# Traneptora/hydrium

Measured on AMD Instinct MI355X. Metric: Mpixel/s encode (8K RGB, default q), higher is better.
Workload: dtype f32

## Files before the change

### hydrium_amd/csrc/hip/device_api.hip

```cpp
#include <hip/hip_runtime.h>

#include <stdint.h>
#include <stdio.h>
#include <stdlib.h>
#include <string.h>

#include <atomic>
#include <condition_variable>
#include <functional>
#include <mutex>
#include <thread>
#include <vector>

#include "../../../include/hydrium_amd.h"
#include "hydk_common.h"
#include "../hyd_sample_fmt.h"

#pragma clang fp contract(off)

namespace hydk {
hipError_t launch_transform(const HydkLfJob *d_jobs, int num_slots, unsigned fmt_mask, int xmode, uint32_t *status,
                            uint2 *part_info, int plog, hipStream_t stream);
hipError_t launch_tables(const uint32_t *hist, HydkTables *tabs, const uint32_t *alpha_max, int nclusters, int first_slot,
                         int num_slots, uint32_t alpha_floor, const uint32_t *alpha_floor_dev, const uint32_t *lf_hist,
// ... 5 lines not shown
hipError_t launch_rans(const HydkLfJob *d_jobs, const uint32_t *sym_count, const HydkTables *tabs, uint32_t *bitbuf,
                       uint32_t bit_pitch_words, uint32_t *group_bits, int num_slots, const uint32_t *status,
                       hipStream_t stream);
hipError_t launch_rans_deferred(const HydkLfJob *d_jobs, const uint32_t *sym_count, const HydkTables *tabs, uint16_t *aux,
                                uint16_t *flags, uint32_t aux_pitch, uint32_t *final_state, uint32_t *group_bits,
                                int num_slots, const uint32_t *status, hipStream_t stream);
hipError_t launch_rans_lanes(const HydkLfJob *d_jobs, const uint32_t *sym_count, const HydkTables *tabs, uint16_t *aux,
                             uint16_t *flags, uint32_t aux_pitch, uint32_t *final_state, uint32_t *group_bits,
                             int nclusters, int num_slots, const uint32_t *status, const uint32_t *lf_hist,
                             HydkLfStream *lf_streams, void *lf_work, hipStream_t stream);
hipError_t launch_lf_front(const HydkLfJob *d_jobs, unsigned long long *recs, uint32_t *hist, void *work, int num_slots,
                           hipStream_t stream);
hipError_t launch_lf_back(const HydkLfJob *d_jobs, const unsigned long long *recs, HydkLfStream *streams, uint32_t *bits,
                          void *work, int num_slots, hipStream_t stream);
hipError_t launch_rans_emit(const HydkLfJob *d_jobs, const uint32_t *sym_count, const uint16_t *aux, const uint16_t *flags,
                            uint32_t aux_pitch, const uint32_t *final_state, const uint32_t *group_bits, const uint64_t *offsets,
                            uint8_t *payload, int num_slots, const uint32_t *status, hipStream_t stream);
hipError_t launch_frame_begin(const HydkLfJob *host_jobs, HydkLfJob *d_jobs, int count, uint32_t *accum, size_t accum_words,
                              hipStream_t stream);
hipError_t launch_publish(const uint64_t *total, uint64_t *h_total, const unsigned long long *lf_total,
                          unsigned long long *h_lf_total, const uint32_t *status, uint32_t *h_status, hipStream_t stream);
hipError_t transform_footprint(int fmt, int storage, int xmode, int *lds_bytes, int *registers);
hipError_t launch_scan(const uint32_t *group_bits, int count, uint64_t *offsets, uint64_t *total, uint8_t *payload,
                       uint64_t payload_cap, int clear_shared_words, uint32_t *status, hipStream_t stream);
hipError_t launch_pack(const uint32_t *bitbuf, uint32_t bit_pitch_words, const uint32_t *group_bits, const uint64_t *offsets,
                       uint8_t *payload, int count, const uint32_t *status, hipStream_t stream);
size_t lf_work_bytes();
hipError_t launch_batch_extents(const void *blob, int frames, void *extents, hipStream_t stream);
hipError_t launch_lf_coder(const HydkLfJob *d_jobs, unsigned long long *recs, uint32_t *hist, HydkLfStream *streams,
                           uint32_t *bits, void *work, int num_slots, hipStream_t stream);
hipError_t launch_lf_gather(HydkLfStream *streams, const uint32_t *bits, uint32_t *packed, unsigned long long *total,
                            int num_slots, hipStream_t stream);
// ... 43 lines not shown
    int linear_light = 0;
    int use_luts = 2;
    int best_register_mode = 2;
    int curve_gathers = 0;
    uint64_t published_pixels = 0;
    uint64_t seen_bytes = 0, seen_pixels = 0;
    int register_luts_ok = 0;
    int rans_lanes = 0;
    uint32_t tok_cap = HYDK_DEFAULT_TOKEN_CAP;
    bool caps_forced = false;
    unsigned grown_ahead = 0;
    uint32_t rec_bytes = 4;
    uint32_t bit_pitch_words = 0;
    int want_transform = 0, want_entropy = 0;
    bool slot_lanes[HYDAMD_MAX_LF_GROUPS] = {};
    unsigned overflow_reruns = 0;
    uint32_t alpha_floor = 0;
    const uint32_t *alpha_floor_dev = nullptr;
    unsigned num_presets = 1;
    int scheme = 0;
    int nclusters = 9;
    hipStream_t own_stream = nullptr;
    hipStream_t stream = nullptr;
    char error[256] = "";

    char *tokens = nullptr;
    uint32_t *bitbuf = nullptr;
    uint16_t *rans_aux = nullptr;
    uint16_t *rans_flags = nullptr;
    uint32_t *rans_final = nullptr;
// ... 1975 lines not shown
                                                 ctx->lf_streams + first, ctx->lf_work + (size_t)first * hydk::lf_work_bytes(),
                                                 ctx->stream));
        } else if (!any_float && wave_form_defers()) {
            HIP_TRY(ctx, hydk::launch_rans_deferred(jobs, ctx->sym_count + g0, ctx->tables + first, ctx->rans_aux + g0 * ctx->tok_cap,
                                                    ctx->rans_flags + g0 * (ctx->tok_cap / 16), ctx->tok_cap, ctx->rans_final + g0,
                                                    ctx->group_bits + g0, count, ctx->status, ctx->stream));
            emits = true;
        } else {
            const int st = ensure_bitbuf(ctx);
            if (st != ST_OK)
                return st;
            HIP_TRY(ctx, hydk::launch_rans(jobs, ctx->sym_count + g0, ctx->tables + first,
                                           ctx->bitbuf + g0 * ctx->bit_pitch_words, ctx->bit_pitch_words,
                                           ctx->group_bits + g0, count, ctx->status, ctx->stream));
        }
        for (int i = first; i < first + count; i++)
            ctx->slot_lanes[i] = emits;
    }
    return ST_OK;
}

int hydamd_run_entropy(HydAmdContext *ctx, int num_slots) {
    if (!ctx)
        return ST_API_ERROR;
    if (num_slots < 1 || num_slots > ctx->max_slots)
        return fail(ctx, ST_API_ERROR, "slot count out of range");
    if (num_slots > ctx->transformed)
        return fail(ctx, ST_API_ERROR, "the entropy stage needs the transform stage of the same slots first");
    HIP_TRY(ctx, hipSetDevice(ctx->device));
    const int count = num_slots * HYDK_GROUPS_PER_LFG;
    ctx->results_valid = false;
    ctx->want_entropy = num_slots;
// ... 9 lines not shown
            ScopedTimer timer(ctx, HYDAMD_K_LF);
            if (!(lf_drop() & 1))
            HIP_TRY(ctx, hydk::launch_lf_front(ctx->d_jobs + lf_first, ctx->lf_recs + (size_t)lf_first * HYDK_LF_SYMBOLS,
                                               ctx->lf_hist + (size_t)lf_first * HYDK_LF_CODES,
                                               ctx->lf_work + (size_t)lf_first * hydk::lf_work_bytes(), lf_count, ctx->stream));
        }
    }
    if (num_slots > ctx->coded) {
        const int st = entropy_range(ctx, ctx->coded, num_slots - ctx->coded, lf_count > 0 && !(lf_drop() & 2));
        if (st != ST_OK)
            return st;
        ctx->coded = num_slots;
    }
    if (!(debug_skip() & 4)) {
        ScopedTimer timer(ctx, HYDAMD_K_PACK);
        HIP_TRY(ctx, hydk::launch_scan(ctx->group_bits, count, ctx->offsets, ctx->total, ctx->payload, ctx->payload_cap, 1,
                                       ctx->status, ctx->stream));
        for (int first = 0; first < num_slots;) {
            int last = first;
            while (last + 1 < num_slots && ctx->slot_lanes[last + 1] == ctx->slot_lanes[first])
                last++;
            const int n = last - first + 1;
            const size_t g0 = (size_t)first * HYDK_GROUPS_PER_LFG;
            if (ctx->slot_lanes[first])
                HIP_TRY(ctx, hydk::launch_rans_emit(ctx->d_jobs + first, ctx->sym_count + g0, ctx->rans_aux + g0 * ctx->tok_cap,
                                                    ctx->rans_flags + g0 * (ctx->tok_cap / 16), ctx->tok_cap,
                                                    ctx->rans_final + g0, ctx->group_bits + g0, ctx->offsets + g0, ctx->payload,
                                                    n, ctx->status, ctx->stream));
            else
                HIP_TRY(ctx, hydk::launch_pack(ctx->bitbuf + g0 * ctx->bit_pitch_words, ctx->bit_pitch_words,
                                               ctx->group_bits + g0, ctx->offsets + g0, ctx->payload,
                                               n * HYDK_GROUPS_PER_LFG, ctx->status, ctx->stream));
            first = last + 1;
        }
    }
    if (lf_count > 0) {
        ScopedTimer timer(ctx, HYDAMD_K_LF);
        if (!(lf_drop() & 4))
        HIP_TRY(ctx, hydk::launch_lf_back(ctx->d_jobs + lf_first, ctx->lf_recs + (size_t)lf_first * HYDK_LF_SYMBOLS,
                                          ctx->lf_streams + lf_first, ctx->lf_bits + (size_t)lf_first * HYDK_LF_BITWORDS,
                                          ctx->lf_work + (size_t)lf_first * hydk::lf_work_bytes(), lf_count, ctx->stream));
        ctx->lf_coded = num_slots;
        ctx->lf_need_gather = true;
// ... 322 lines not shown
    if (run_pairs)
        *run_pairs = h.run_pairs;
    if (bit_count)
        *bit_count = h.bit_count;
    return ST_OK;
}

int hydamd_read_lf_bits(HydAmdContext *ctx, int slot, uint8_t *dst, size_t capacity) {
    int st = check_slot(ctx, slot);
    if (st != ST_OK)
        return st;
    if (!ctx->lf_on_device || !ctx->lf_results_valid)
        return fail(ctx, ST_API_ERROR, "no device-coded LF stream: the LF coder is off or the frame was not synchronised");
    if (capacity > (size_t)HYDK_LF_BITWORDS * sizeof(uint32_t))
        return fail(ctx, ST_API_ERROR, "LF bit request too large");
    if (capacity)
        HIP_TRY(ctx, hipMemcpy(dst, ctx->lf_bits + (size_t)slot * HYDK_LF_BITWORDS, capacity, hipMemcpyDeviceToHost));
    return ST_OK;
}

size_t hydamd_lf_payload_size(HydAmdContext *ctx) {
    return ctx && ctx->lf_results_valid && ctx->lf_on_device ? (size_t)ctx->h_lf_total : 0;
}

const uint8_t *hydamd_lf_payload_device(HydAmdContext *ctx) { return ctx ? (const uint8_t *)ctx->lf_packed : nullptr; }

int hydamd_read_lf_payload(HydAmdContext *ctx, uint8_t *dst, size_t capacity) {
    if (!ctx || !ctx->lf_on_device || !ctx->lf_results_valid)
        return fail(ctx, ST_API_ERROR, "no device-coded LF stream: the LF coder is off or the frame was not synchronised");
    if (capacity < ctx->h_lf_total)
        return fail(ctx, ST_API_ERROR, "LF payload buffer too small");
    if (ctx->h_lf_total)
// ... 159 lines not shown
```

### hydrium_amd/csrc/hip/kernels.hip

```cpp
#include <hip/hip_runtime.h>
#include <stdint.h>

#include "hydk_common.h"
#include <atomic>
#include <type_traits>

#pragma clang fp contract(off)

namespace {

constexpr int kThreads = 256;
#ifndef HYDK_K1_WAVES
#define HYDK_K1_WAVES 4
#endif
#ifndef HYDK_K1_GATHER
#define HYDK_K1_GATHER 0x10
#endif
#ifndef HYDK_K1_WAVELOCAL
#define HYDK_K1_WAVELOCAL 1
#endif
#ifndef HYDK_K1_SKIP
#define HYDK_K1_SKIP 0
#endif
#ifndef HYDK_K1_ILP
// ... 1148 lines not shown
        if (bogus)
            atomicOr(status, HYDK_STATUS_INCONSISTENT);
    }
}

__global__ __launch_bounds__(kThreads) void k_build_tables(const uint32_t *hist_all, HydkTables *tabs,
                                                           const uint32_t *alpha_max_all, int nclusters,
                                                           uint32_t alpha_floor, const uint32_t *alpha_floor_dev,
                                                           int first_slot, int num_slots, const uint32_t *lf_hist,
                                                           HydkLfStream *lf_streams, void *lf_work, const HydkLfJob *__restrict__ jobs_all) {
    HYDK_URGENT();
    if ((int)blockIdx.x >= num_slots) {
        __shared__ LfHuffScratch s_huff;
        const int s = (int)blockIdx.x - num_slots;
        if (threadIdx.x < 64)
            lf_huffman_wave(lf_hist + (size_t)s * HYDK_LF_CODES, ((LfWork *)lf_work)[s].codes, lf_streams + s, s_huff, (int)threadIdx.x);
        return;
    }
    const unsigned slot = (unsigned)first_slot + blockIdx.x;
    const uint32_t *hist = hist_all + (size_t)slot * HYDK_MAX_CLUSTERS * HYDK_ALPHABET;
    HydkTables *tab = tabs + slot;
    __shared__ uint32_t s_freq[HYDK_MAX_CLUSTERS][HYDK_ALPHABET];
    __shared__ uint32_t s_cutoff[HYDK_MAX_CLUSTERS][HYDK_ALPHABET];
    __shared__ uint32_t s_other[HYDK_MAX_CLUSTERS][HYDK_ALPHABET];
    __shared__ uint32_t s_shift[HYDK_MAX_CLUSTERS][HYDK_ALPHABET];
    __shared__ uint32_t s_base[HYDK_MAX_CLUSTERS][HYDK_ALPHABET];
    __shared__ uint8_t s_under[HYDK_MAX_CLUSTERS][HYDK_ALPHABET];
    __shared__ uint8_t s_over[HYDK_MAX_CLUSTERS][HYDK_ALPHABET];
    __shared__ uint32_t s_alpha[HYDK_MAX_CLUSTERS];
    __shared__ uint32_t s_log_alpha, s_err;

// ... 527 lines not shown
    unsigned char *const s_tab = s_mem + kOpsBytes;
    __builtin_amdgcn_s_setprio(HYDK_CHAIN_PRIO);
#if HYDK_CHAIN_DYN_LDS
    if ((uint32_t)(uintptr_t)(__attribute__((address_space(3))) unsigned char *)s_mem != 0u)
        __builtin_trap();
#endif
#if HYDK_CHAIN_PROBE & 32
    const uint32_t probe_t0 = (uint32_t)__builtin_amdgcn_s_memrealtime();
#endif
#if HYDK_CHAIN_HOG
    asm volatile("v_accvgpr_write_b32 a255, 0" ::: "a255");
#endif
    const int lane = threadIdx.x;
    if ((int)blockIdx.x >= num_slots) {
        const int s = (int)blockIdx.x - num_slots;
        lf_huffman_wave(lf_hist + (size_t)s * HYDK_LF_CODES, ((LfWork *)lf_work)[s].codes, lf_streams + s, *(LfHuffScratch *)s_mem, lane);
        return;
    }
    const int slot = blockIdx.x;
    const int ngroups = jobs[slot].gcols * jobs[slot].grows;
    const HydkTables *tab = tabs + slot;
    if (*status & HYDK_STATUS_OVERFLOW)
        return;
    typedef __attribute__((address_space(3))) const uint16_t LdsU16;
    {
#if HYDK_LANE_TAB_GLOBAL
        const uint32_t tab_lds = 0;
#else
        const uint4 *src = (const uint4 *)&tab->inv1[0][0];
        for (int i = lane; i < NC * HYDK_ANS_SLOTS / 8; i += 64)
            ((uint4 *)s_tab)[i] = src[i];
// ... 384 lines not shown
#if HYDK_CHAIN_PROBE & 32
    if (lane == 0)
        group_bits_all[G] = probe_t0;
    if (lane == 1)
        group_bits_all[G] = (uint32_t)__builtin_amdgcn_s_memrealtime();
#endif
}

#ifndef HYDK_EMIT_SHARE_DEFAULT
#define HYDK_EMIT_SHARE_DEFAULT 1
#endif
constexpr int kEmitPer = 8;
constexpr int kEmitBatch = 64 * kEmitPer;
constexpr int kEmitWin = kEmitBatch + 4;

__global__ __launch_bounds__(kThreads) void k_rans_emit(const HydkLfJob *__restrict__ jobs, const uint32_t *sym_count_all,
                                                        const uint16_t *aux_all, const uint16_t *flags_all, uint32_t aux_pitch,
                                                        const uint32_t *final_state_all, const uint32_t *group_bits_all,
                                                        const uint64_t *offsets_all, uint8_t *payload,
                                                        const uint32_t *status, int vblocks) {
    __shared__ uint32_t s_win[4][kEmitWin];
    HYDK_URGENT();
    const int t = threadIdx.x, lane = t & 63, wave = t >> 6;
    auto one_block = [&](const int vb) {
    const int slot = vb >> 4;
    const int g = ((vb & 15) << 2) + wave;
    const int ngroups = jobs[slot].gcols * jobs[slot].grows;
    const size_t G = (size_t)slot * HYDK_GROUPS_PER_LFG + g;
    if (g >= ngroups || (*status & HYDK_STATUS_OVERFLOW))
        return;
    const void *tok = (const char *)jobs[slot].tokens + (size_t)g * jobs[slot].tok_cap * jobs[slot].rec_bytes;
    const uint4 *aux = (const uint4 *)(aux_all + G * aux_pitch);
    const uint16_t *flags = flags_all + G * (aux_pitch / 16);
    uint32_t *W = (uint32_t *)payload;
    uint32_t *win = s_win[wave];
    const int n = __builtin_amdgcn_readfirstlane((int)sym_count_all[G]);
    const uint32_t bits = group_bits_all[G];
    const unsigned long long lo_bit = offsets_all[G] * 8ull, hi_bit = lo_bit + (unsigned long long)((bits + 7u) & ~7u);
    const uint32_t shared_lo = (lo_bit & 31ull) ? (uint32_t)(lo_bit >> 5) : 0xFFFFFFFFu;
    const uint32_t shared_hi = (hi_bit & 31ull) ? (uint32_t)((hi_bit - 1ull) >> 5) : 0xFFFFFFFFu;
    const uint32_t wbase = (uint32_t)(lo_bit >> 5);
    uint32_t cur = (uint32_t)(lo_bit & 31ull) + bits;
    uint32_t carry = 0;

    bool bad = false;
    auto put = [&](uint32_t word, uint32_t v) {
        const uint32_t d = wbase + word;
        if (d == shared_lo || d == shared_hi)
            atomicOr(&W[d], v);
        else
            W[d] = v;
    };
    auto emit = [&](const uint32_t (&val)[kEmitPer], const uint32_t (&nb)[kEmitPer], auto &&before_stores) {
        uint32_t mine = 0;
#pragma unroll
        for (int j = 0; j < kEmitPer; j++)
            mine += nb[j];
        const uint32_t inc = scan64_inclusive(mine);
        const uint32_t total = __builtin_amdgcn_readlane(inc, 63);
        if (!total) {
            before_stores();
            return;
        }
        if (total > cur) {
            if (lane == 0)
                atomicOr((uint32_t *)status, HYDK_STATUS_INCONSISTENT);
            bad = true;
            return;
        }
        const uint32_t newcur = cur - total;
        const uint32_t wlo = newcur >> 5, whi = (cur - 1u) >> 5;
        const uint32_t nwords = whi - wlo + 1u;
        for (uint32_t i = lane; i < nwords; i += 64)
            win[i] = 0;
        __builtin_amdgcn_wave_barrier();
        if (lane == 0 && (cur & 31u))
            win[whi - wlo] = carry;
        __builtin_amdgcn_wave_barrier();
        uint32_t pos = newcur + (inc - mine) - wlo * 32u;
#pragma unroll
        for (int j = 0; j < kEmitPer; j++) {
// ... 416 lines not shown
    if (nclusters == 9)
        HYDK_LAUNCH_LANES(HYDK_LANE_NC9_PROBE);
    else if (nclusters == 3)
        HYDK_LAUNCH_LANES(3);
    else if (nclusters == 2)
        HYDK_LAUNCH_LANES(2);
    else if (nclusters == 1)
        HYDK_LAUNCH_LANES(1);
    else
        return hipErrorInvalidValue;
#undef HYDK_LAUNCH_LANES
    return hipGetLastError();
}

hipError_t launch_rans_emit(const HydkLfJob *d_jobs, const uint32_t *sym_count, const uint16_t *aux, const uint16_t *flags,
                            uint32_t aux_pitch, const uint32_t *final_state, const uint32_t *group_bits, const uint64_t *offsets,
                            uint8_t *payload, int num_slots, const uint32_t *status, hipStream_t stream) {
    static const int share = [] {
        const char *v = getenv("HYDAMD_EMIT_SHARE");
        const int n = v && *v ? atoi(v) : HYDK_EMIT_SHARE_DEFAULT;
        return n < 1 ? 1 : n > 16 ? 16 : n;
    }();
    const int vblocks = num_slots * 16;
    hipLaunchKernelGGL(k_rans_emit, dim3((vblocks + share - 1) / share), dim3(kThreads), 0, stream, d_jobs, sym_count, aux, flags,
                       aux_pitch, final_state, group_bits, offsets, payload, status, vblocks);
    return hipGetLastError();
}

hipError_t launch_frame_begin(const HydkLfJob *host_jobs, HydkLfJob *d_jobs, int count, uint32_t *accum, size_t accum_words,
                              hipStream_t stream) {
    const uint32_t quads = accum ? (uint32_t)(accum_words / 4) : 0u;
    const uint32_t job_words = (uint32_t)((size_t)count * sizeof(HydkLfJob) / sizeof(uint32_t));
    const uint32_t blocks = 1u + (quads + kThreads - 1) / kThreads;
    hipLaunchKernelGGL(k_frame_begin, dim3(blocks < 64u ? blocks : 64u), dim3(kThreads), 0, stream, (const uint32_t *)host_jobs,
                       (uint32_t *)d_jobs, job_words, (uint4 *)accum, quads);
    return hipGetLastError();
}

hipError_t launch_publish(const uint64_t *total, uint64_t *h_total, const unsigned long long *lf_total,
                          unsigned long long *h_lf_total, const uint32_t *status, uint32_t *h_status, hipStream_t stream) {
// ... 40 lines not shown
```

### hydrium_amd/csrc/hip/lf_coder.hip

```cpp
#include <hip/hip_runtime.h>

#include <stdint.h>

#include "hydk_common.h"
#ifndef HYDK_LF_WPB
#define HYDK_LF_WPB 1
#endif
#ifndef HYDK_LF_PROBE
#define HYDK_LF_PROBE 0
#endif

namespace {

#include "lf_huffman.h"

constexpr int kPlane = HYDK_DC_PITCH * HYDK_DC_PITCH;

#define LF_REC(v, lit, r) ((unsigned long long)(v) | ((unsigned long long)((uint32_t)(lit) | ((uint32_t)(r) << 1)) << 32))

struct LfShape {
    int vbw, blocks, n;
    uint32_t vbw_magic;
};

__device__ __forceinline__ LfShape lf_shape(const HydkLfJob &job) {
    LfShape sh;
    sh.vbw = (job.width + 7) >> 3;
    sh.blocks = sh.vbw * ((job.height + 7) >> 3);
    sh.n = 3 * sh.blocks;
    sh.vbw_magic = sh.vbw > 1 ? (uint32_t)(0xFFFFFFFFu / (uint32_t)sh.vbw) + 1u : 0u;
    return sh;
}

__device__ __forceinline__ int lf_row_of(const LfShape &sh, int rem) {
    return sh.vbw > 1 ? (int)__umulhi((uint32_t)rem, sh.vbw_magic) : rem;
}

__device__ __forceinline__ void lf_hybrid(uint32_t v, uint32_t &token, uint32_t &nbits, uint32_t &residue) {
    if (v < 128u) {
        token = v;
        nbits = 0;
        residue = 0;
        return;
    }
    const uint32_t nb = (31u - (uint32_t)__clz(v)) - 2u;
    residue = (v >> 1) & ((1u << nb) - 1u);
    token = 128u + (((nb - 5u) << 2) | (((v >> (nb + 1u)) & 1u) << 1) | (v & 1u));
    nbits = nb;
}

#define LF_DPP_KEEP(v, ctrl, rmask) ((uint32_t)__builtin_amdgcn_update_dpp((int)(v), (int)(v), ctrl, rmask, 0xF, false))
#define LF_DPP_ZERO(v, ctrl, rmask) ((uint32_t)__builtin_amdgcn_update_dpp(0, (int)(v), ctrl, rmask, 0xF, false))

__device__ __forceinline__ int wave_incl_max(int v) {
    int t;
    t = (int)LF_DPP_KEEP(v, 0x111, 0xF);
    v = v > t ? v : t;
    t = (int)LF_DPP_KEEP(v, 0x112, 0xF);
    v = v > t ? v : t;
    t = (int)LF_DPP_KEEP(v, 0x114, 0xF);
    v = v > t ? v : t;
    t = (int)LF_DPP_KEEP(v, 0x118, 0xF);
    v = v > t ? v : t;
    t = (int)LF_DPP_KEEP(v, 0x142, 0xA);
    v = v > t ? v : t;
    t = (int)LF_DPP_KEEP(v, 0x143, 0xC);
    v = v > t ? v : t;
    return v;
}

__device__ __forceinline__ uint32_t wave_incl_sum(uint32_t v) {
    v += LF_DPP_ZERO(v, 0x111, 0xF);
    v += LF_DPP_ZERO(v, 0x112, 0xF);
    v += LF_DPP_ZERO(v, 0x114, 0xF);
    v += LF_DPP_ZERO(v, 0x118, 0xF);
    v += LF_DPP_ZERO(v, 0x142, 0xA);
    v += LF_DPP_ZERO(v, 0x143, 0xC);
    return v;
}

struct LfTokenScratch {
    int wtot[kLfWaves];
    uint32_t lastv[kLfWaves];
    int head[kLfWaves];
    uint32_t first;
};

__device__ __forceinline__ uint32_t lf_predict(int32_t cur, int32_t w, int32_t n, int32_t nw) {
    const int32_t lo = w < n ? w : n, hi = w < n ? n : w;
    int32_t pred = (int32_t)((uint32_t)w + (uint32_t)n - (uint32_t)nw);
    pred = pred < lo ? lo : pred > hi ? hi : pred;
    const uint32_t d = (uint32_t)cur - (uint32_t)pred;
// ... 235 lines not shown
    const HydkLfJob &job = jobs[slot];
    const LfShape sh = lf_shape(job);
    __shared__ __attribute__((aligned(16))) int s_rs[kScanSpan];
    __shared__ uint32_t s_hist[HYDK_LF_CODES];
    __shared__ LfTokenScratch s_tok;
    __shared__ uint32_t s_rbits;
    if (HYDK_LF_PROBE & 8)
        return;
    for (int win = (int)blockIdx.x * HYDK_LF_WPB; win < ((int)blockIdx.x + 1) * HYDK_LF_WPB && win < kMaxWindows; win++) {
        const int tb = win * kEmitSpan;
        if (tb >= sh.n)
            return;
        if (tid == 0)
            s_rbits = 0;
        uint32_t rb = lf_tokens_window(job, sh, recs_all + (size_t)slot * HYDK_LF_SYMBOLS, tb, s_rs, s_hist, s_tok);
        rb = wave_incl_sum(rb);
        if ((tid & 63) == 63 && rb)
            atomicAdd(&s_rbits, rb);
        __syncthreads();
        LfWork &w = work[slot];
        for (int i = tid; i < HYDK_LF_CODES && !(HYDK_LF_PROBE & 2); i += kLfThreads) {
            const uint32_t c = s_hist[i];
            w.win_hist[win][i] = (uint16_t)c;
            if (c)
                atomicAdd(&hist_all[(size_t)slot * HYDK_LF_CODES + i], c);
        }
        if (tid == 0)
            w.win_residue_bits[win] = s_rbits;
        if (HYDK_LF_WPB > 1)
            __syncthreads();
    }
}

__global__ __launch_bounds__(64) void k_lf_codes(const uint32_t *__restrict__ hist_all, HydkLfStream *__restrict__ streams,
                                                 LfWork *__restrict__ work) {
    if (!(HYDK_LF_PROBE & 1))
        __builtin_amdgcn_s_setprio(3);
    __shared__ LfHuffScratch s_huff;
    const int slot = blockIdx.x;
    lf_huffman_wave(hist_all + (size_t)slot * HYDK_LF_CODES, work[slot].codes, streams + slot, s_huff, (int)threadIdx.x);
}

__global__ __launch_bounds__(kLfThreads) void k_lf_offsets(const HydkLfJob *__restrict__ jobs, LfWork *__restrict__ work,
                                                           HydkLfStream *__restrict__ streams, uint32_t *__restrict__ bits_all) {
    if (!(HYDK_LF_PROBE & 1))
        __builtin_amdgcn_s_setprio(3);
    const int slot = blockIdx.x, tid = threadIdx.x, lane = tid & 63, wave = tid >> 6;
    const LfShape sh = lf_shape(jobs[slot]);
    const int windows = (sh.n + kEmitSpan - 1) / kEmitSpan;
    LfWork &w = work[slot];
    __shared__ uint32_t s_win[kMaxWindows];
    __shared__ uint32_t s_wsum[kLfWaves];
    uint32_t len6[6];
#pragma unroll
    for (int j = 0; j < 6; j++)
        len6[j] = w.codes[j * 64 + lane] >> 16;
    for (int win = wave; win < windows; win += kLfWaves) {
        uint32_t bits = 0;
#pragma unroll
        for (int j = 0; j < 6; j++)
            bits += (uint32_t)w.win_hist[win][j * 64 + lane] * len6[j];
        bits = wave_incl_sum(bits);
        if (lane == 63)
            s_win[win] = bits + w.win_residue_bits[win];
    }
    __syncthreads();
    const uint32_t mine = tid < windows ? s_win[tid] : 0u;
    const uint32_t inc = wave_incl_sum(mine);
    if (lane == 63)
        s_wsum[wave] = inc;
    __syncthreads();
    uint32_t off = inc - mine, total = 0;
    for (int k = 0; k < kLfWaves; k++) {
        if (k < wave)
            off += s_wsum[k];
        total += s_wsum[k];
    }
    uint32_t *out = bits_all + (size_t)slot * HYDK_LF_BITWORDS;
    if (tid < windows) {
        w.win_off[tid] = off;
        if (mine) {
            out[off >> 5] = 0;
            out[(off + mine - 1u) >> 5] = 0;
        }
    }
    if (tid == 0)
        streams[slot].bit_count = total;
}

__global__ __launch_bounds__(kLfThreads) void k_lf_pack(const HydkLfJob *__restrict__ jobs,
                                                        const unsigned long long *__restrict__ recs_all,
                                                        const LfWork *__restrict__ work, uint32_t *__restrict__ bits_all) {
    if (!(HYDK_LF_PROBE & 1))
        __builtin_amdgcn_s_setprio(3);
    const int slot = blockIdx.y, tid = threadIdx.x, lane = tid & 63, wave = tid >> 6;
    const LfShape sh = lf_shape(jobs[slot]);
    __shared__ uint32_t s_bits[kPackWords];
    __shared__ uint32_t s_code[HYDK_LF_CODES];
    __shared__ uint32_t s_wsum[kLfWaves];
    if ((int)blockIdx.x * HYDK_LF_WPB * kEmitSpan >= sh.n)
        return;
    for (int i = tid; i < HYDK_LF_CODES; i += kLfThreads)
        s_code[i] = work[slot].codes[i];
  for (int win = (int)blockIdx.x * HYDK_LF_WPB; win < ((int)blockIdx.x + 1) * HYDK_LF_WPB && win < kMaxWindows; win++) {
    const int tb = win * kEmitSpan;
    if (tb >= sh.n)
        return;
    if (win != (int)blockIdx.x * HYDK_LF_WPB)
        __syncthreads();
    for (int w = tid; w < kPackWords; w += kLfThreads)
        s_bits[w] = 0;
    __syncthreads();
    unsigned long long val[4];
    uint32_t len[4];
    const uint32_t mine = lf_window_strings(sh, recs_all + (size_t)slot * HYDK_LF_SYMBOLS, tb, s_code, val, len);
    const uint32_t inc = wave_incl_sum(mine);
    if (lane == 63)
        s_wsum[wave] = inc;
    __syncthreads();
    const uint32_t gbits = work[slot].win_off[win];
    uint32_t pos = (gbits & 31u) + inc - mine, total = 0;
    for (int w = 0; w < kLfWaves; w++) {
        const uint32_t t = s_wsum[w];
        if (w < wave)
            pos += t;
        total += t;
    }
#pragma unroll
    for (int j = 0; j < 4; j++) {
        if (!len[j])
            continue;
        const uint32_t w = pos >> 5, shl = pos & 31u;
        const unsigned long long lo = val[j] << shl;
        const uint32_t hi = shl ? (uint32_t)(val[j] >> (64u - shl)) : 0u;
        if ((uint32_t)lo)
            atomicOr(&s_bits[w], (uint32_t)lo);
        if ((uint32_t)(lo >> 32))
            atomicOr(&s_bits[w + 1], (uint32_t)(lo >> 32));
        if (hi)
            atomicOr(&s_bits[w + 2], hi);
        pos += len[j];
    }
    __syncthreads();
    if (!total)
        continue;
    const uint32_t end = (gbits & 31u) + total, last = (end - 1u) >> 5;
    uint32_t *dst = bits_all + (size_t)slot * HYDK_LF_BITWORDS + (gbits >> 5);
    for (uint32_t w = tid; w <= last; w += kLfThreads) {
        if (w == 0 || w == last)
            atomicOr(&dst[w], s_bits[w]);
        else
            dst[w] = s_bits[w];
    }
  }
}

__global__ __launch_bounds__(256) void k_lf_gather(HydkLfStream *__restrict__ streams, const uint32_t *__restrict__ bits_all,
                                                   uint32_t *__restrict__ packed, unsigned long long *__restrict__ total,
                                                   int num_slots) {
    const int slot = blockIdx.x, tid = threadIdx.x;
    __shared__ uint32_t s_off;
    if (tid < 64) {
        uint32_t mine = 0;
        for (int s = tid; s < slot; s += 64)
            mine += (streams[s].bit_count + 31u) >> 5;
#pragma unroll
        for (int d = 32; d >= 1; d >>= 1)
// ... 4 lines not shown
    __syncthreads();
    const uint32_t off = s_off, words = (streams[slot].bit_count + 31u) >> 5;
    const uint32_t *src = bits_all + (size_t)slot * HYDK_LF_BITWORDS;
    for (uint32_t w = tid; w < words; w += 256)
        packed[off + w] = src[w];
    if (tid == 0) {
        streams[slot].offset = off * 4u;
        if (slot == num_slots - 1)
            *total = (unsigned long long)(off + words) * 4ull;
    }
}

__global__ __launch_bounds__(64) void k_lf_huffman(const uint32_t *__restrict__ hist, HydkLfStream *__restrict__ stream_out,
                                                   uint32_t *__restrict__ codes) {
    __shared__ LfHuffScratch s_huff;
    lf_huffman_wave(hist, codes, stream_out, s_huff, (int)threadIdx.x);
}

}

namespace hydk {

size_t lf_work_bytes() { return sizeof(LfWork); }

hipError_t launch_lf_front(const HydkLfJob *d_jobs, unsigned long long *recs, uint32_t *hist, void *work, int num_slots,
                           hipStream_t stream) {
    hipLaunchKernelGGL(k_lf_tokens, dim3((kMaxWindows + HYDK_LF_WPB - 1) / HYDK_LF_WPB, num_slots), dim3(kLfThreads), 0, stream, d_jobs, recs, hist, (LfWork *)work);
    return hipGetLastError();
}

hipError_t launch_lf_codes(const uint32_t *hist, HydkLfStream *streams, void *work, int num_slots, hipStream_t stream) {
    hipLaunchKernelGGL(k_lf_codes, dim3(num_slots), dim3(64), 0, stream, hist, streams, (LfWork *)work);
    return hipGetLastError();
}

hipError_t launch_lf_back(const HydkLfJob *d_jobs, const unsigned long long *recs, HydkLfStream *streams, uint32_t *bits,
                          void *work, int num_slots, hipStream_t stream) {
    LfWork *w = (LfWork *)work;
    hipLaunchKernelGGL(k_lf_offsets, dim3(num_slots), dim3(kLfThreads), 0, stream, d_jobs, w, streams, bits);
    hipLaunchKernelGGL(k_lf_pack, dim3((kMaxWindows + HYDK_LF_WPB - 1) / HYDK_LF_WPB, num_slots), dim3(kLfThreads), 0, stream, d_jobs, recs, w, bits);
    return hipGetLastError();
}

hipError_t launch_lf_coder(const HydkLfJob *d_jobs, unsigned long long *recs, uint32_t *hist, HydkLfStream *streams,
                           uint32_t *bits, void *work, int num_slots, hipStream_t stream) {
    hipError_t e = launch_lf_front(d_jobs, recs, hist, work, num_slots, stream);
    if (e == hipSuccess)
        e = launch_lf_codes(hist, streams, work, num_slots, stream);
    if (e == hipSuccess)
        e = launch_lf_back(d_jobs, recs, streams, bits, work, num_slots, stream);
    return e;
}

hipError_t launch_lf_gather(HydkLfStream *streams, const uint32_t *bits, uint32_t *packed, unsigned long long *total,
                            int num_slots, hipStream_t stream) {
    hipLaunchKernelGGL(k_lf_gather, dim3(num_slots), dim3(256), 0, stream, streams, bits, packed, total, num_slots);
    return hipGetLastError();
}

hipError_t launch_lf_huffman_only(const uint32_t *hist, HydkLfStream *stream_out, uint32_t *codes, hipStream_t stream) {
    hipLaunchKernelGGL(k_lf_huffman, dim3(1), dim3(64), 0, stream, hist, stream_out, codes);
    return hipGetLastError();
}
// ... 3 lines not shown
```

### hydrium_amd/csrc/hip/lf_huffman.h

```cpp
#ifndef HYDK_LF_HUFFMAN_H_
#define HYDK_LF_HUFFMAN_H_

constexpr int kLfThreads = 256;
constexpr int kLfWaves = kLfThreads / 64;
constexpr int kScanSpan = kLfThreads * 4;
constexpr int kAhead = 128;
constexpr int kEmitSpan = kScanSpan - kAhead;
constexpr int kMaxWindows = (HYDK_LF_SYMBOLS + kEmitSpan - 1) / kEmitSpan;

struct LfWork {
    uint32_t codes[HYDK_LF_CODES];
    uint32_t win_residue_bits[kMaxWindows];
    uint32_t win_off[kMaxWindows];
    uint16_t win_hist[kMaxWindows][HYDK_LF_CODES];
};
__device__ __forceinline__ void wave_sync() {
    __builtin_amdgcn_fence(__ATOMIC_RELEASE, "wavefront");
    __builtin_amdgcn_wave_barrier();
    __builtin_amdgcn_fence(__ATOMIC_ACQUIRE, "wavefront");
}

constexpr int kRunLo = 768, kMergedLo = 896;
constexpr int kMaxDepth = 15;

// ... 35 lines not shown
    const unsigned long long m = __ballot(has);
    any = m != 0;
    return any ? (uint32_t)__builtin_amdgcn_readlane((int)v, __builtin_ctzll(m)) : 0u;
}

__device__ __forceinline__ int clog2_i(int v) { return v <= 1 ? 0 : 32 - __clz(v - 1); }

struct LfHuffScratch {
    uint16_t par[2 * HYDK_LF_CODES];
    uint16_t depth[2 * HYDK_LF_CODES];
    uint32_t cnt[16], first[16];
    uint32_t err;
};

__device__ __forceinline__ void lf_huffman_wave(const uint32_t *hist, uint32_t *codes, HydkLfStream *st, LfHuffScratch &S,
                                                int lane) {
    const unsigned long long ltmask = (1ull << lane) - 1ull;
    uint16_t *s_par = S.par, *s_depth = S.depth;
    uint32_t *s_cnt = S.cnt, *s_first = S.first;
    uint32_t &s_err = S.err;

    if (lane < 16)
        s_cnt[lane] = 0;
    if (lane == 0)
        s_err = 0;

    uint32_t ek[kEntries], em[kEntries], f6[kEntries];
    int maxidx = -1, live0 = 0;
    uint32_t pairs = 0, total = 0;
#pragma unroll
    for (int t = 0; t < kEntries; t++) {
// ... 96 lines not shown
            s_par[M_WHO(fm)] = (uint16_t)k;
            s_par[M_WHO(sm)] = (uint16_t)k;
        }
        merges = k + 1;
    }
    if (!err && live0 - merges != 1)
        err = 3;
    wave_sync();

    if (lane == 0 && merges > 0) {
        s_depth[HYDK_LF_CODES + merges - 1] = 0;
        for (int m = merges - 2; m >= 0; m--)
            s_depth[HYDK_LF_CODES + m] = (uint16_t)(s_depth[HYDK_LF_CODES + s_par[HYDK_LF_CODES + m]] + 1);
    }
    wave_sync();
    uint32_t len6[6];
#pragma unroll
    for (int j = 0; j < 6; j++) {
        const int ci = j * 64 + lane;
        uint32_t len = 0;
        if (f6[j] && merges > 0 && !err)
            len = (uint32_t)s_depth[HYDK_LF_CODES + s_par[ci]] + 1u;
        if (len > (uint32_t)kMaxDepth) {
            err = 4;
            len = 0;
        }
        len6[j] = len;
        if (len)
            atomicAdd(&s_cnt[len], 1u);
    }
    wave_sync();
// ... 23 lines not shown
            if (len6[j] == (uint32_t)L)
                code = run[L] + (uint32_t)__popcll(m & ltmask);
            run[L] += (uint32_t)__popcll(m);
        }
        const uint32_t len = len6[j];
        codes[ci] = len ? (len << 16) | (__brev(code) >> (32u - len)) : 0u;
        st->lengths[ci] = (uint8_t)len;
    }
    if (lane == 0) {
        st->alphabet = (uint32_t)n;
        st->run_pairs = pairs;
        st->error = s_err;
    }
}


#endif
```

Before: 98950.

## Fold payload scan into rANS emit and LF offsets into Huffman wave

When every slot uses the lane-chain rANS path, the separate scan kernel is skipped. A self-scanning variant of the emit kernel instead computes each group's byte offset, the total and the overflow status itself, and stores boundary words with byte masks rather than atomics. On the LF side, the k_lf_offsets kernel is removed and its per-window bit offsets are computed inside the Huffman code wave, which cuts a kernel launch. The trade-off is redundant work: every emit wave re-sums all preceding group sizes, which is O(G) per group, and the window-offset pass now runs serially on a single wave. The diff also adds masked edge stores in LF pack and a bounded LF bit readback.

```diff
diff --git a/hydrium_amd/csrc/hip/device_api.hip b/hydrium_amd/csrc/hip/device_api.hip
--- a/hydrium_amd/csrc/hip/device_api.hip
+++ b/hydrium_amd/csrc/hip/device_api.hip
@@ -43,8 +43,9 @@
 hipError_t launch_lf_back(const HydkLfJob *d_jobs, const unsigned long long *recs, HydkLfStream *streams, uint32_t *bits,
                           void *work, int num_slots, hipStream_t stream);
 hipError_t launch_rans_emit(const HydkLfJob *d_jobs, const uint32_t *sym_count, const uint16_t *aux, const uint16_t *flags,
-                            uint32_t aux_pitch, const uint32_t *final_state, const uint32_t *group_bits, const uint64_t *offsets,
-                            uint8_t *payload, int num_slots, const uint32_t *status, hipStream_t stream);
+                            uint32_t aux_pitch, const uint32_t *final_state, const uint32_t *group_bits, uint64_t *offsets,
+                            uint8_t *payload, int num_slots, uint32_t *status, uint64_t *total, uint64_t payload_cap,
+                            hipStream_t stream);
 hipError_t launch_frame_begin(const HydkLfJob *host_jobs, HydkLfJob *d_jobs, int count, uint32_t *accum, size_t accum_words,
                               hipStream_t stream);
 hipError_t launch_publish(const uint64_t *total, uint64_t *h_total, const unsigned long long *lf_total,
@@ -118,6 +119,7 @@
     uint32_t bit_pitch_words = 0;
     int want_transform = 0, want_entropy = 0;
     bool slot_lanes[HYDAMD_MAX_LF_GROUPS] = {};
+    bool slot_lane_chain[HYDAMD_MAX_LF_GROUPS] = {};
     unsigned overflow_reruns = 0;
     uint32_t alpha_floor = 0;
     const uint32_t *alpha_floor_dev = nullptr;
@@ -2123,8 +2125,10 @@
                                            ctx->bitbuf + g0 * ctx->bit_pitch_words, ctx->bit_pitch_words,
                                            ctx->group_bits + g0, count, ctx->status, ctx->stream));
         }
-        for (int i = first; i < first + count; i++)
+        for (int i = first; i < first + count; i++) {
             ctx->slot_lanes[i] = emits;
+            ctx->slot_lane_chain[i] = lanes;
+        }
     }
     return ST_OK;
 }
@@ -2164,9 +2168,17 @@
     }
     if (!(debug_skip() & 4)) {
         ScopedTimer timer(ctx, HYDAMD_K_PACK);
-        HIP_TRY(ctx, hydk::launch_scan(ctx->group_bits, count, ctx->offsets, ctx->total, ctx->payload, ctx->payload_cap, 1,
-                                       ctx->status, ctx->stream));
-        for (int first = 0; first < num_slots;) {
+        bool all_emit = true;
+        for (int i = 0; i < num_slots; i++)
+            all_emit = all_emit && ctx->slot_lane_chain[i];
+        if (all_emit)
+            HIP_TRY(ctx, hydk::launch_rans_emit(ctx->d_jobs, ctx->sym_count, ctx->rans_aux, ctx->rans_flags, ctx->tok_cap,
+                                                ctx->rans_final, ctx->group_bits, ctx->offsets, ctx->payload, num_slots,
+                                                ctx->status, ctx->total, ctx->payload_cap, ctx->stream));
+        else
+            HIP_TRY(ctx, hydk::launch_scan(ctx->group_bits, count, ctx->offsets, ctx->total, ctx->payload, ctx->payload_cap, 1,
+                                           ctx->status, ctx->stream));
+        for (int first = all_emit ? num_slots : 0; first < num_slots;) {
             int last = first;
             while (last + 1 < num_slots && ctx->slot_lanes[last + 1] == ctx->slot_lanes[first])
                 last++;
@@ -2176,7 +2188,7 @@
                 HIP_TRY(ctx, hydk::launch_rans_emit(ctx->d_jobs + first, ctx->sym_count + g0, ctx->rans_aux + g0 * ctx->tok_cap,
                                                     ctx->rans_flags + g0 * (ctx->tok_cap / 16), ctx->tok_cap,
                                                     ctx->rans_final + g0, ctx->group_bits + g0, ctx->offsets + g0, ctx->payload,
-                                                    n, ctx->status, ctx->stream));
+                                                    n, ctx->status, nullptr, 0, ctx->stream));
             else
                 HIP_TRY(ctx, hydk::launch_pack(ctx->bitbuf + g0 * ctx->bit_pitch_words, ctx->bit_pitch_words,
                                                ctx->group_bits + g0, ctx->offsets + g0, ctx->payload,
@@ -2529,8 +2541,14 @@
         return fail(ctx, ST_API_ERROR, "no device-coded LF stream: the LF coder is off or the frame was not synchronised");
     if (capacity > (size_t)HYDK_LF_BITWORDS * sizeof(uint32_t))
         return fail(ctx, ST_API_ERROR, "LF bit request too large");
-    if (capacity)
-        HIP_TRY(ctx, hipMemcpy(dst, ctx->lf_bits + (size_t)slot * HYDK_LF_BITWORDS, capacity, hipMemcpyDeviceToHost));
+    if (!capacity)
+        return ST_OK;
+    HydkLfStream h;
+    HIP_TRY(ctx, hipMemcpy(&h, ctx->lf_streams + slot, sizeof(h), hipMemcpyDeviceToHost));
+    const size_t have = ((size_t)h.bit_count + 7u) / 8u, n = capacity < have ? capacity : have;
+    if (n)
+        HIP_TRY(ctx, hipMemcpy(dst, ctx->lf_bits + (size_t)slot * HYDK_LF_BITWORDS, n, hipMemcpyDeviceToHost));
+    memset(dst + n, 0, capacity - n);
     return ST_OK;
 }
 
diff --git a/hydrium_amd/csrc/hip/hydk_edges.h b/hydrium_amd/csrc/hip/hydk_edges.h
--- /dev/null
+++ b/hydrium_amd/csrc/hip/hydk_edges.h
@@ -0,0 +1,31 @@
+#ifndef HYD_SECTION_EDGES_H_
+#define HYD_SECTION_EDGES_H_
+
+#include <stdint.h>
+
+#ifdef __HIPCC__
+#define HYDK_EDGE_FN __host__ __device__ static inline
+#else
+#define HYDK_EDGE_FN static inline
+#endif
+
+HYDK_EDGE_FN uint32_t hydk_edge_byte_mask(uint64_t word, uint64_t lo_byte, uint64_t hi_byte) {
+    const uint64_t w0 = word * 4u, w1 = w0 + 4u;
+    const uint64_t a = lo_byte > w0 ? lo_byte : w0, b = hi_byte < w1 ? hi_byte : w1;
+    if (a >= b)
+        return 0u;
+    return (0xFu >> (4u - (uint32_t)(b - a))) << (uint32_t)(a - w0);
+}
+
+HYDK_EDGE_FN void hydk_store_edge_word(uint8_t *payload, uint64_t word, uint32_t v, uint64_t lo_byte, uint64_t hi_byte) {
+    const uint32_t mask = hydk_edge_byte_mask(word, lo_byte, hi_byte);
+    if (mask == 0xFu) {
+        *(uint32_t *)(payload + word * 4u) = v;
+        return;
+    }
+    for (uint32_t b = 0; b < 4u; b++)
+        if ((mask >> b) & 1u)
+            payload[word * 4u + b] = (uint8_t)(v >> (8u * b));
+}
+
+#endif
diff --git a/hydrium_amd/csrc/hip/kernels.hip b/hydrium_amd/csrc/hip/kernels.hip
--- a/hydrium_amd/csrc/hip/kernels.hip
+++ b/hydrium_amd/csrc/hip/kernels.hip
@@ -2,6 +2,7 @@
 #include <stdint.h>
 
 #include "hydk_common.h"
+#include "hydk_edges.h"
 #include <atomic>
 #include <type_traits>
 
@@ -1186,7 +1187,8 @@
         __shared__ LfHuffScratch s_huff;
         const int s = (int)blockIdx.x - num_slots;
         if (threadIdx.x < 64)
-            lf_huffman_wave(lf_hist + (size_t)s * HYDK_LF_CODES, ((LfWork *)lf_work)[s].codes, lf_streams + s, s_huff, (int)threadIdx.x);
+            lf_code_and_offsets_wave(lf_hist + (size_t)s * HYDK_LF_CODES, ((LfWork *)lf_work)[s], lf_streams + s,
+                                     jobs_all[first_slot + s], s_huff, (int)threadIdx.x);
         return;
     }
     const unsigned slot = (unsigned)first_slot + blockIdx.x;
@@ -1744,7 +1746,8 @@
     const int lane = threadIdx.x;
     if ((int)blockIdx.x >= num_slots) {
         const int s = (int)blockIdx.x - num_slots;
-        lf_huffman_wave(lf_hist + (size_t)s * HYDK_LF_CODES, ((LfWork *)lf_work)[s].codes, lf_streams + s, *(LfHuffScratch *)s_mem, lane);
+        lf_code_and_offsets_wave(lf_hist + (size_t)s * HYDK_LF_CODES, ((LfWork *)lf_work)[s], lf_streams + s, jobs[s],
+                                 *(LfHuffScratch *)s_mem, lane);
         return;
     }
     const int slot = blockIdx.x;
@@ -2159,20 +2162,54 @@
 constexpr int kEmitBatch = 64 * kEmitPer;
 constexpr int kEmitWin = kEmitBatch + 4;
 
+template <bool SELF>
 __global__ __launch_bounds__(kThreads) void k_rans_emit(const HydkLfJob *__restrict__ jobs, const uint32_t *sym_count_all,
                                                         const uint16_t *aux_all, const uint16_t *flags_all, uint32_t aux_pitch,
                                                         const uint32_t *final_state_all, const uint32_t *group_bits_all,
-                                                        const uint64_t *offsets_all, uint8_t *payload,
-                                                        const uint32_t *status, int vblocks) {
+                                                        uint64_t *offsets_all, uint8_t *payload, uint32_t *status, int vblocks,
+                                                        uint64_t *total, uint64_t payload_cap) {
     __shared__ uint32_t s_win[4][kEmitWin];
     HYDK_URGENT();
     const int t = threadIdx.x, lane = t & 63, wave = t >> 6;
+    auto wave_sum = [](uint64_t v) {
+        const uint32_t lo = __builtin_amdgcn_readlane(scan64_inclusive((uint32_t)v & 0xFFFFFFu), 63);
+        const uint32_t hi = __builtin_amdgcn_readlane(scan64_inclusive((uint32_t)(v >> 24)), 63);
+        return ((uint64_t)hi << 24) + lo;
+    };
+    uint64_t all = 0;
+    bool fits = true;
+    if (SELF) {
+        uint64_t mine_all = 0;
+        for (int i = lane; i < vblocks * 4; i += 64)
+            mine_all += (group_bits_all[i] + 7u) >> 3;
+        all = wave_sum(mine_all);
+        fits = all <= payload_cap && !(*status & HYDK_STATUS_OVERFLOW);
+    }
     auto one_block = [&](const int vb) {
     const int slot = vb >> 4;
     const int g = ((vb & 15) << 2) + wave;
     const int ngroups = jobs[slot].gcols * jobs[slot].grows;
     const size_t G = (size_t)slot * HYDK_GROUPS_PER_LFG + g;
-    if (g >= ngroups || (*status & HYDK_STATUS_OVERFLOW))
+    uint64_t sec_lo = 0;
+    if (SELF) {
+        uint64_t mine_before = 0;
+        for (size_t i = lane; i < G; i += 64)
+            mine_before += (group_bits_all[i] + 7u) >> 3;
+        sec_lo = wave_sum(mine_before);
+        if (lane == 0) {
+            offsets_all[G] = sec_lo;
+            if (G == 0) {
+                *total = fits ? all : 0;
+                if (all > payload_cap)
+                    atomicOr(status, HYDK_STATUS_PAYLOAD);
+                if (fits)
+                    for (uint64_t b = all; b & 3u; b++)
+                        payload[b] = 0;
+            }
+        }
+        if (g >= ngroups || !fits)
+            return;
+    } else if (g >= ngroups || (*status & HYDK_STATUS_OVERFLOW))
         return;
     const void *tok = (const char *)jobs[slot].tokens + (size_t)g * jobs[slot].tok_cap * jobs[slot].rec_bytes;
     const uint4 *aux = (const uint4 *)(aux_all + G * aux_pitch);
@@ -2181,7 +2218,7 @@
     uint32_t *win = s_win[wave];
     const int n = __builtin_amdgcn_readfirstlane((int)sym_count_all[G]);
     const uint32_t bits = group_bits_all[G];
-    const unsigned long long lo_bit = offsets_all[G] * 8ull, hi_bit = lo_bit + (unsigned long long)((bits + 7u) & ~7u);
+    const unsigned long long lo_bit = (SELF ? sec_lo : offsets_all[G]) * 8ull, hi_bit = lo_bit + (unsigned long long)((bits + 7u) & ~7u);
     const uint32_t shared_lo = (lo_bit & 31ull) ? (uint32_t)(lo_bit >> 5) : 0xFFFFFFFFu;
     const uint32_t shared_hi = (hi_bit & 31ull) ? (uint32_t)((hi_bit - 1ull) >> 5) : 0xFFFFFFFFu;
     const uint32_t wbase = (uint32_t)(lo_bit >> 5);
@@ -2191,7 +2228,9 @@
     bool bad = false;
     auto put = [&](uint32_t word, uint32_t v) {
         const uint32_t d = wbase + word;
-        if (d == shared_lo || d == shared_hi)
+        if (SELF && (d == shared_lo || d == shared_hi))
+            hydk_store_edge_word(payload, d, v, lo_bit >> 3, hi_bit >> 3);
+        else if (d == shared_lo || d == shared_hi)
             atomicOr(&W[d], v);
         else
             W[d] = v;
@@ -2209,7 +2248,7 @@
         }
         if (total > cur) {
             if (lane == 0)
-                atomicOr((uint32_t *)status, HYDK_STATUS_INCONSISTENT);
+                atomicOr(status, HYDK_STATUS_INCONSISTENT);
             bad = true;
             return;
         }
@@ -2656,16 +2695,22 @@
 }
 
 hipError_t launch_rans_emit(const HydkLfJob *d_jobs, const uint32_t *sym_count, const uint16_t *aux, const uint16_t *flags,
-                            uint32_t aux_pitch, const uint32_t *final_state, const uint32_t *group_bits, const uint64_t *offsets,
-                            uint8_t *payload, int num_slots, const uint32_t *status, hipStream_t stream) {
+                            uint32_t aux_pitch, const uint32_t *final_state, const uint32_t *group_bits, uint64_t *offsets,
+                            uint8_t *payload, int num_slots, uint32_t *status, uint64_t *total, uint64_t payload_cap,
+                            hipStream_t stream) {
     static const int share = [] {
         const char *v = getenv("HYDAMD_EMIT_SHARE");
         const int n = v && *v ? atoi(v) : HYDK_EMIT_SHARE_DEFAULT;
         return n < 1 ? 1 : n > 16 ? 16 : n;
     }();
     const int vblocks = num_slots * 16;
-    hipLaunchKernelGGL(k_rans_emit, dim3((vblocks + share - 1) / share), dim3(kThreads), 0, stream, d_jobs, sym_count, aux, flags,
-                       aux_pitch, final_state, group_bits, offsets, payload, status, vblocks);
+    const dim3 grid((vblocks + share - 1) / share);
+    if (total)
+        hipLaunchKernelGGL(k_rans_emit<true>, grid, dim3(kThreads), 0, stream, d_jobs, sym_count, aux, flags, aux_pitch, final_state,
+                           group_bits, offsets, payload, status, vblocks, total, payload_cap);
+    else
+        hipLaunchKernelGGL(k_rans_emit<false>, grid, dim3(kThreads), 0, stream, d_jobs, sym_count, aux, flags, aux_pitch,
+                           final_state, group_bits, offsets, payload, status, vblocks, (uint64_t *)nullptr, (uint64_t)0);
     return hipGetLastError();
 }
 
diff --git a/hydrium_amd/csrc/hip/lf_coder.hip b/hydrium_amd/csrc/hip/lf_coder.hip
--- a/hydrium_amd/csrc/hip/lf_coder.hip
+++ b/hydrium_amd/csrc/hip/lf_coder.hip
@@ -27,7 +27,7 @@
     LfShape sh;
     sh.vbw = (job.width + 7) >> 3;
     sh.blocks = sh.vbw * ((job.height + 7) >> 3);
-    sh.n = 3 * sh.blocks;
+    sh.n = lf_values_of(job);
     sh.vbw_magic = sh.vbw > 1 ? (uint32_t)(0xFFFFFFFFu / (uint32_t)sh.vbw) + 1u : 0u;
     return sh;
 }
@@ -50,7 +50,6 @@
 }
 
 #define LF_DPP_KEEP(v, ctrl, rmask) ((uint32_t)__builtin_amdgcn_update_dpp((int)(v), (int)(v), ctrl, rmask, 0xF, false))
-#define LF_DPP_ZERO(v, ctrl, rmask) ((uint32_t)__builtin_amdgcn_update_dpp(0, (int)(v), ctrl, rmask, 0xF, false))
 
 __device__ __forceinline__ int wave_incl_max(int v) {
     int t;
@@ -66,16 +65,6 @@
     v = v > t ? v : t;
     t = (int)LF_DPP_KEEP(v, 0x143, 0xC);
     v = v > t ? v : t;
-    return v;
-}
-
-__device__ __forceinline__ uint32_t wave_incl_sum(uint32_t v) {
-    v += LF_DPP_ZERO(v, 0x111, 0xF);
-    v += LF_DPP_ZERO(v, 0x112, 0xF);
-    v += LF_DPP_ZERO(v, 0x114, 0xF);
-    v += LF_DPP_ZERO(v, 0x118, 0xF);
-    v += LF_DPP_ZERO(v, 0x142, 0xA);
-    v += LF_DPP_ZERO(v, 0x143, 0xC);
     return v;
 }
 
@@ -341,7 +330,7 @@
         if (tid == 0)
             s_rbits = 0;
         uint32_t rb = lf_tokens_window(job, sh, recs_all + (size_t)slot * HYDK_LF_SYMBOLS, tb, s_rs, s_hist, s_tok);
-        rb = wave_incl_sum(rb);
+        rb = lf_wave_incl_sum(rb);
         if ((tid & 63) == 63 && rb)
             atomicAdd(&s_rbits, rb);
         __syncthreads();
@@ -359,65 +348,19 @@
     }
 }
 
-__global__ __launch_bounds__(64) void k_lf_codes(const uint32_t *__restrict__ hist_all, HydkLfStream *__restrict__ streams,
-                                                 LfWork *__restrict__ work) {
+__global__ __launch_bounds__(64) void k_lf_codes(const HydkLfJob *__restrict__ jobs, const uint32_t *__restrict__ hist_all,
+                                                 HydkLfStream *__restrict__ streams, LfWork *__restrict__ work) {
     if (!(HYDK_LF_PROBE & 1))
         __builtin_amdgcn_s_setprio(3);
     __shared__ LfHuffScratch s_huff;
     const int slot = blockIdx.x;
-    lf_huffman_wave(hist_all + (size_t)slot * HYDK_LF_CODES, work[slot].codes, streams + slot, s_huff, (int)threadIdx.x);
-}
-
-__global__ __launch_bounds__(kLfThreads) void k_lf_offsets(const HydkLfJob *__restrict__ jobs, LfWork *__restrict__ work,
-                                                           HydkLfStream *__restrict__ streams, uint32_t *__restrict__ bits_all) {
-    if (!(HYDK_LF_PROBE & 1))
-        __builtin_amdgcn_s_setprio(3);
-    const int slot = blockIdx.x, tid = threadIdx.x, lane = tid & 63, wave = tid >> 6;
-    const LfShape sh = lf_shape(jobs[slot]);
-    const int windows = (sh.n + kEmitSpan - 1) / kEmitSpan;
-    LfWork &w = work[slot];
-    __shared__ uint32_t s_win[kMaxWindows];
-    __shared__ uint32_t s_wsum[kLfWaves];
-    uint32_t len6[6];
-#pragma unroll
-    for (int j = 0; j < 6; j++)
-        len6[j] = w.codes[j * 64 + lane] >> 16;
-    for (int win = wave; win < windows; win += kLfWaves) {
-        uint32_t bits = 0;
-#pragma unroll
-        for (int j = 0; j < 6; j++)
-            bits += (uint32_t)w.win_hist[win][j * 64 + lane] * len6[j];
-        bits = wave_incl_sum(bits);
-        if (lane == 63)
-            s_win[win] = bits + w.win_residue_bits[win];
-    }
-    __syncthreads();
-    const uint32_t mine = tid < windows ? s_win[tid] : 0u;
-    const uint32_t inc = wave_incl_sum(mine);
-    if (lane == 63)
-        s_wsum[wave] = inc;
-    __syncthreads();
-    uint32_t off = inc - mine, total = 0;
-    for (int k = 0; k < kLfWaves; k++) {
-        if (k < wave)
-            off += s_wsum[k];
-        total += s_wsum[k];
-    }
-    uint32_t *out = bits_all + (size_t)slot * HYDK_LF_BITWORDS;
-    if (tid < windows) {
-        w.win_off[tid] = off;
-        if (mine) {
-            out[off >> 5] = 0;
-            out[(off + mine - 1u) >> 5] = 0;
-        }
-    }
-    if (tid == 0)
-        streams[slot].bit_count = total;
+    lf_code_and_offsets_wave(hist_all + (size_t)slot * HYDK_LF_CODES, work[slot], streams + slot, jobs[slot], s_huff, (int)threadIdx.x);
 }
 
 __global__ __launch_bounds__(kLfThreads) void k_lf_pack(const HydkLfJob *__restrict__ jobs,
                                                         const unsigned long long *__restrict__ recs_all,
-                                                        const LfWork *__restrict__ work, uint32_t *__restrict__ bits_all) {
+                                                        const LfWork *__restrict__ work,
+                                                        const HydkLfStream *__restrict__ streams, uint32_t *__restrict__ bits_all) {
     if (!(HYDK_LF_PROBE & 1))
         __builtin_amdgcn_s_setprio(3);
     const int slot = blockIdx.y, tid = threadIdx.x, lane = tid & 63, wave = tid >> 6;
@@ -441,7 +384,7 @@
     unsigned long long val[4];
     uint32_t len[4];
     const uint32_t mine = lf_window_strings(sh, recs_all + (size_t)slot * HYDK_LF_SYMBOLS, tb, s_code, val, len);
-    const uint32_t inc = wave_incl_sum(mine);
+    const uint32_t inc = lf_wave_incl_sum(mine);
     if (lane == 63)
         s_wsum[wave] = inc;
     __syncthreads();
@@ -472,12 +415,22 @@
     if (!total)
         continue;
     const uint32_t end = (gbits & 31u) + total, last = (end - 1u) >> 5;
+    if ((gbits >> 5) + last >= (uint32_t)HYDK_LF_BITWORDS)
+        continue;
+    const bool ends_stream = gbits + total == streams[slot].bit_count;
     uint32_t *dst = bits_all + (size_t)slot * HYDK_LF_BITWORDS + (gbits >> 5);
     for (uint32_t w = tid; w <= last; w += kLfThreads) {
-        if (w == 0 || w == last)
+        uint32_t mask = 0xFFFFFFFFu;
+        if (w == 0)
+            mask <<= gbits & 31u;
+        if (w == last && (end & 31u) && !ends_stream)
+            mask &= (1u << (end & 31u)) - 1u;
+        if (mask == 0xFFFFFFFFu)
+            dst[w] = s_bits[w];
+        else {
+            atomicAnd(&dst[w], ~mask);
             atomicOr(&dst[w], s_bits[w]);
-        else
-            dst[w] = s_bits[w];
+        }
     }
   }
 }
@@ -512,7 +465,8 @@
 __global__ __launch_bounds__(64) void k_lf_huffman(const uint32_t *__restrict__ hist, HydkLfStream *__restrict__ stream_out,
                                                    uint32_t *__restrict__ codes) {
     __shared__ LfHuffScratch s_huff;
-    lf_huffman_wave(hist, codes, stream_out, s_huff, (int)threadIdx.x);
+    uint32_t len6[kEntries];
+    lf_huffman_wave(hist, codes, stream_out, s_huff, (int)threadIdx.x, len6);
 }
 
 }
@@ -527,16 +481,17 @@
     return hipGetLastError();
 }
 
-hipError_t launch_lf_codes(const uint32_t *hist, HydkLfStream *streams, void *work, int num_slots, hipStream_t stream) {
-    hipLaunchKernelGGL(k_lf_codes, dim3(num_slots), dim3(64), 0, stream, hist, streams, (LfWork *)work);
+hipError_t launch_lf_codes(const HydkLfJob *d_jobs, const uint32_t *hist, HydkLfStream *streams, void *work, int num_slots,
+                           hipStream_t stream) {
+    hipLaunchKernelGGL(k_lf_codes, dim3(num_slots), dim3(64), 0, stream, d_jobs, hist, streams, (LfWork *)work);
     return hipGetLastError();
 }
 
 hipError_t launch_lf_back(const HydkLfJob *d_jobs, const unsigned long long *recs, HydkLfStream *streams, uint32_t *bits,
                           void *work, int num_slots, hipStream_t stream) {
     LfWork *w = (LfWork *)work;
-    hipLaunchKernelGGL(k_lf_offsets, dim3(num_slots), dim3(kLfThreads), 0, stream, d_jobs, w, streams, bits);
-    hipLaunchKernelGGL(k_lf_pack, dim3((kMaxWindows + HYDK_LF_WPB - 1) / HYDK_LF_WPB, num_slots), dim3(kLfThreads), 0, stream, d_jobs, recs, w, bits);
+    hipLaunchKernelGGL(k_lf_pack, dim3((kMaxWindows + HYDK_LF_WPB - 1) / HYDK_LF_WPB, num_slots), dim3(kLfThreads), 0, stream, d_jobs, recs, w,
+                       streams, bits);
     return hipGetLastError();
 }
 
@@ -544,7 +499,7 @@
                            uint32_t *bits, void *work, int num_slots, hipStream_t stream) {
     hipError_t e = launch_lf_front(d_jobs, recs, hist, work, num_slots, stream);
     if (e == hipSuccess)
-        e = launch_lf_codes(hist, streams, work, num_slots, stream);
+        e = launch_lf_codes(d_jobs, hist, streams, work, num_slots, stream);
     if (e == hipSuccess)
         e = launch_lf_back(d_jobs, recs, streams, bits, work, num_slots, stream);
     return e;
diff --git a/hydrium_amd/csrc/hip/lf_huffman.h b/hydrium_amd/csrc/hip/lf_huffman.h
--- a/hydrium_amd/csrc/hip/lf_huffman.h
+++ b/hydrium_amd/csrc/hip/lf_huffman.h
@@ -73,7 +73,7 @@
 };
 
 __device__ __forceinline__ void lf_huffman_wave(const uint32_t *hist, uint32_t *codes, HydkLfStream *st, LfHuffScratch &S,
-                                                int lane) {
+                                                int lane, uint32_t (&len6)[kEntries]) {
     const unsigned long long ltmask = (1ull << lane) - 1ull;
     uint16_t *s_par = S.par, *s_depth = S.depth;
     uint32_t *s_cnt = S.cnt, *s_first = S.first;
@@ -200,7 +200,6 @@
             s_depth[HYDK_LF_CODES + m] = (uint16_t)(s_depth[HYDK_LF_CODES + s_par[HYDK_LF_CODES + m]] + 1);
     }
     wave_sync();
-    uint32_t len6[6];
 #pragma unroll
     for (int j = 0; j < 6; j++) {
         const int ci = j * 64 + lane;
@@ -254,5 +253,58 @@
     }
 }
 
+#define LF_DPP_ADD(v, ctrl, rmask) ((v) + (uint32_t)__builtin_amdgcn_update_dpp(0, (int)(v), ctrl, rmask, 0xF, false))
+__device__ __forceinline__ uint32_t lf_wave_incl_sum(uint32_t v) {
+    v = LF_DPP_ADD(v, 0x111, 0xF);
+    v = LF_DPP_ADD(v, 0x112, 0xF);
+    v = LF_DPP_ADD(v, 0x114, 0xF);
+    v = LF_DPP_ADD(v, 0x118, 0xF);
+    v = LF_DPP_ADD(v, 0x142, 0xA);
+    v = LF_DPP_ADD(v, 0x143, 0xC);
+    return v;
+}
+
+__device__ __forceinline__ void lf_window_offsets_wave(const uint32_t (&len6)[kEntries], LfWork &w, HydkLfStream *st, int windows,
+                                                       int lane) {
+    uint32_t carry = 0;
+#pragma unroll
+    for (int k = 0; k < (kMaxWindows + 63) / 64; k++) {
+        uint32_t mine = 0;
+#pragma unroll 4
+        for (int i = 0; i < 64; i++) {
+            if (k * 64 + i >= windows)
+                continue;
+            const uint16_t *row = w.win_hist[k * 64 + i];
+            uint32_t bits = 0;
+#pragma unroll
+            for (int j = 0; j < kEntries; j++)
+                bits += (uint32_t)row[j * 64 + lane] * len6[j];
+            bits = (uint32_t)__builtin_amdgcn_readlane((int)lf_wave_incl_sum(bits), 63);
+            mine = lane == i ? bits : mine;
+        }
+        const bool has = k * 64 + lane < windows;
+        if (has)
+            mine += w.win_residue_bits[k * 64 + lane];
+        const uint32_t inc = lf_wave_incl_sum(mine);
+        if (has)
+            w.win_off[k * 64 + lane] = carry + inc - mine;
+        carry += (uint32_t)__builtin_amdgcn_readlane((int)inc, 63);
+    }
+    if (lane == 0)
+        st->bit_count = carry;
+}
+
+__device__ __forceinline__ int lf_values_of(const HydkLfJob &job) {
+    return 3 * ((job.width + 7) >> 3) * ((job.height + 7) >> 3);
+}
+__device__ __forceinline__ int lf_windows_of(const HydkLfJob &job) { return (lf_values_of(job) + kEmitSpan - 1) / kEmitSpan; }
+
+__device__ __forceinline__ void lf_code_and_offsets_wave(const uint32_t *hist, LfWork &w, HydkLfStream *st, const HydkLfJob &job,
+                                                         LfHuffScratch &S, int lane) {
+    uint32_t len6[kEntries];
+    lf_huffman_wave(hist, w.codes, st, S, lane, len6);
+    lf_window_offsets_wave(len6, w, st, lf_windows_of(job), lane);
+}
+
 
 #endif
```

Result: faster. 100,800, median of 6 (+1.8%).
